# dkohlsdorf/audio_pattern_discovery

Measured on AMD Instinct MI355X. Metric: DTW cell-updates/sec (whole node), higher is better.
Workload: dtype f32

## Files before the change

audio_pattern_discovery_amd/csrc/dtw_systolic.h:

```cpp
#pragma once
#include <type_traits>

#ifndef APD_ABLATE
#define APD_ABLATE 0
#endif

#include "dtw_common.h"

namespace apd {

typedef float apd_f32x4 __attribute__((ext_vector_type(4)));
constexpr uint32_t kNoFrame = 0xFFFFFF00u;

template <int D>
__device__ __forceinline__ void load_frame(float (&dst)[D], __amdgpu_buffer_rsrc_t rsrc, uint32_t byte_off)
{
    constexpr int DP4 = (D + 3) / 4;
#pragma unroll
    for (int q = 0; q < DP4; ++q) {
        const apd_f32x4 t = __builtin_bit_cast(apd_f32x4, __builtin_amdgcn_raw_buffer_load_b128(rsrc, byte_off + 16u * q, 0, 0));
        if (4 * q + 0 < D) dst[4 * q + 0] = t.x;
        if (4 * q + 1 < D) dst[4 * q + 1] = t.y;
        if (4 * q + 2 < D) dst[4 * q + 2] = t.z;
        if (4 * q + 3 < D) dst[4 * q + 3] = t.w;
    }
}

template <int D>
__device__ __forceinline__ void load_frame_dwords(float (&dst)[D], __amdgpu_buffer_rsrc_t rsrc, uint32_t byte_off)
{
#pragma unroll
    for (int k = 0; k < D; ++k)
        dst[k] = __builtin_bit_cast(float, __builtin_amdgcn_raw_buffer_load_b32(rsrc, byte_off + 4u * k, 0, 0));
}

template <int D, int DN>
__device__ __forceinline__ float frame_dist(const float (&x)[DN], const float (&y)[DN])
{
    float t = x[0] - y[0];
    float acc = t * t;
#pragma unroll
    for (int k = 1; k < D; ++k) {
        t = x[k] - y[k];
        acc = __builtin_fmaf(t, t, acc);
    }
    if (APD_ABLATE & 1) return acc;
    return __builtin_amdgcn_sqrtf(acc);
}

template <int D, int DN>
__device__ __forceinline__ float frame_sq_strict(const float (&x)[DN], const float (&y)[DN])
{
    float t = x[0] - y[0];
    float acc = t * t;
#pragma unroll
    for (int k = 1; k < D; ++k) {
        t = x[k] - y[k];
        const float sq = t * t;
        acc = acc + sq;
    }
    return acc;
}
template <int D, int DN>
__device__ __forceinline__ float frame_dist_strict(const float (&x)[DN], const float (&y)[DN])
{
    return __builtin_sqrtf(frame_sq_strict<D, DN>(x, y));
}

template <int D>
__device__ __forceinline__ float frame_sq_expanded_pre(const float (&xm)[D + 1], const float (&y)[D + 1])
{
    float acc = xm[D] + y[D];
#pragma unroll
    for (int k = 0; k < D; ++k) acc = __builtin_fmaf(xm[k], y[k], acc);
    return acc;
}
template <int D>
__device__ __forceinline__ void prescale_row_piece(apd_f32x4 &v, int piece)
{
    const bool np = piece == D / 4;
    v.x = (np && D % 4 == 0) ? v.x : -2.0f * v.x;
    v.y = (np && D % 4 == 1) ? v.y : -2.0f * v.y;
    v.z = (np && D % 4 == 2) ? v.z : -2.0f * v.z;
    v.w = (np && D % 4 == 3) ? v.w : -2.0f * v.w;
}
template <int D>
__device__ __forceinline__ float frame_sq_exact_pre(const float (&xm)[D + 1], const float (&y)[D + 1])
{
    float t = __builtin_fmaf(-0.5f, xm[0], -y[0]);
    float acc = t * t;
#pragma unroll
    for (int k = 1; k < D; ++k) {
        t = __builtin_fmaf(-0.5f, xm[k], -y[k]);
        acc = __builtin_fmaf(t, t, acc);
    }
    return acc;
}
template <int C, int G, bool UNIFORM_PEN>
__device__ __forceinline__ void dp_rows_step(float (&prev1)[C], float (&prev2)[C], const float (&d)[C], const bool (&g1)[C],
                                             const bool (&g2)[C], float del, float ins, float mat, int gl)
{
    float left1 = group_from_lower_wrap<G>(prev1[C - 1], APD_INF, gl);
    float left2 = group_from_lower_wrap<G>(prev2[C - 1], APD_INF, gl);
    float upr1 = APD_INF, upr2 = APD_INF;
#pragma unroll
    for (int c = 0; c < C; ++c) {
        if (APD_ABLATE & 2) { prev1[c] += d[c]; prev2[c] -= d[c]; continue; }
        const float up1 = (c < C - 1) ? prev1[(c + 1) % C] : upr1;
        const float up2 = (c < C - 1) ? prev2[(c + 1) % C] : upr2;
        const float r1 = select_node<UNIFORM_PEN>(left1, up1, prev1[c], d[c], del, ins, mat, (APD_ABLATE & 16) ? false : g1[c]);
        const float r2 = select_node<UNIFORM_PEN>(up2, left2, prev2[c], d[c], del, ins, mat, (APD_ABLATE & 16) ? false : g2[c]);
        prev1[c] = r1; prev2[c] = r2;
        left1 = r1; left2 = r2;
        if (c == 0) {
            upr1 = group_from_upper_wrap<G>(r1, APD_INF, gl);
            upr2 = group_from_upper_wrap<G>(r2, APD_INF, gl);
        }
    }
}
template <int C>
__device__ __forceinline__ void slow_phase_captures(float (&prev1)[C], float (&prev2)[C], float &res1, float &res2, int tau, int gl,
                                                    int tau_cap, int cw, int cstar)
{
    if (tau == gl) {
#pragma unroll
        for (int c = 0; c < C; ++c) if (c == cw) { prev1[c] = 0.0f; prev2[c] = 0.0f; }
    }
    if (tau == tau_cap) {
#pragma unroll
        for (int c = 0; c < C; ++c) if (c == cstar) { res1 = prev1[c]; res2 = prev2[c]; }
    }
}
template <int D, int C, int G, bool UNIFORM_PEN, bool HYBRID>
__global__ __launch_bounds__(256) void dtw_fused_systolic(const AlignLaunch L)
{
    static_assert(C >= 2 && (64 % G) == 0, "bad geometry");
    if (L.d_nonfinite != nullptr && *L.d_nonfinite != 0u) return;
    constexpr int DN = D + 1;
    constexpr int DP = (DN + 3) & ~3;
    constexpr int PPW = 64 / G;
    constexpr int WPT = kSlotsPerTile / (4 * PPW);
    const int lane = threadIdx.x & 63;
    const int gl = lane % G;
    const uint32_t xcd = blockIdx.x & 7u, q = blockIdx.x >> 3;
    const uint32_t tile = (q / WPT) * 8u + xcd;
    const uint32_t slot = ((q % WPT) * 4u + (threadIdx.x >> 6)) * PPW + lane / G;
    const PairInfo P = decode_pair(L, tile, slot);
    const bool special = P.valid && (P.n == 1 || P.m == 1);
    const bool sweep = P.valid && !special;
    if (__ballot(sweep) == 0ull) {
        if (special && gl == 0) { const float s = (P.n == 1 && P.m == 1) ? 0.0f : APD_INF; store_pair(L, tile, P, s, s); }
        return;
    }
    const int n = sweep ? P.n : 1, m = sweep ? P.m : 1, w = sweep ? P.w : 2;
    const __amdgpu_buffer_rsrc_t rsrc = __builtin_amdgcn_make_buffer_rsrc((void *)L.d_frames, 0, L.frames_bytes, 0x00020000);
    const uint32_t a_off = (uint32_t)(P.A - L.d_frames) * 4u, b_off = (uint32_t)(P.B - L.d_frames) * 4u;
    constexpr uint32_t FB = DP * 4u;
    float ins = L.band.ins, del = L.band.del, mat = L.band.mat;
    float tau_thr = L.tau, nmax_b = P.nmax_b;
    asm volatile("" : "+v"(ins), "+v"(del), "+v"(mat), "+v"(tau_thr), "+v"(nmax_b));
    constexpr int R = (G == 64) ? 128 : 64;
    constexpr int LPF = DP / 4;
    constexpr int FPF = 64 / LPF;
    constexpr int RS = DP + 4;
    constexpr int U_ROWS = ((C + 1) % 2 == 0) ? (C + 1) : 2 * (C + 1);
    __shared__ float xring_all[4][(R + U_ROWS) * RS];
    float *const xring = xring_all[threadIdx.x >> 6];
    const int lead = __builtin_ctzll(__ballot(sweep));
    const uint32_t a_off_w = __builtin_amdgcn_readlane(a_off, lead);
    const int n_w = __builtin_amdgcn_readlane(n, lead);
    const int u0 = C * gl;
    const int two_w = 2 * w;

    bool g1[C], g2[C];
#pragma unroll
    for (int c = 0; c < C; ++c) {
        const int u = u0 + c;
        g1[c] = u >= two_w;
        g2[c] = (u == 0) | (u > two_w);
    }
    const int cw = w - u0;
    const int ustar = (m - 1) - (n - 1) + w;
    const int cstar = ustar - u0;
    const int tau_cap = (n - 1) + gl;

    const int g_act = (two_w + 1 + C - 1) / C;
    int my_total = sweep ? (n - 1) + g_act : 0;
    int my_min = sweep ? (n - 1) : 0x7fffffff;
    int total = 0, min_rows = 0x7fffffff;
#pragma unroll
    for (int g = 0; g < PPW; ++g) {
        total = max(total, __builtin_amdgcn_readlane(my_total, g * G));
        min_rows = min(min_rows, __builtin_amdgcn_readlane(my_min, g * G));
    }
    constexpr int S = C + 1;
    constexpr int U = (S % 2 == 0) ? S : 2 * S;
    static_assert(U == U_ROWS, "ring copy sized for another unroll");
    constexpr bool MASKED_FETCH = HYBRID && (G == 32 || G == 8) && !(APD_ABLATE & 512);
    const int total_r = ((total + U - 1) / U) * U;
    int a_steps = G;
    if (UNIFORM_PEN && !HYBRID) {
        int w_max = 0;
#pragma unroll
        for (int g = 0; g < PPW; ++g) w_max = max(w_max, __builtin_amdgcn_readlane(w, g * G));
        a_steps = max(G, w_max + 1);
    }
    const int a_end = min(((a_steps + U - 1) / U) * U, total_r);
    const int b_end = min(max((min_rows / U) * U, a_end), total_r);

    float prev1[C], prev2[C];
#pragma unroll
    for (int c = 0; c < C; ++c) { prev1[c] = APD_INF; prev2[c] = APD_INF; }
    float res1 = 0.0f, res2 = 0.0f;

    float yf[S][DN];
#pragma unroll
    for (int c = 0; c < C; ++c) {
        const int j = u0 - gl + c - w;
        const int idx = (j >= 1) ? (min(j, m) - 1) : (HYBRID ? m : m + 1);
        load_frame<DN>(yf[c], rsrc, b_off + (uint32_t)idx * FB);
    }
#pragma unroll
    for (int k = 0; k < DN; ++k) yf[C][k] = 0.0f;
    if (HYBRID && !MASKED_FETCH && !(APD_ABLATE & 8)) {
        const int jt = 1 + (C - 1) * G - w;
        const uint32_t yo = b_off + (uint32_t)((jt >= 1) ? (min(jt, m) - 1) : m) * FB;
        load_frame<DN>(yf[C], rsrc, gl == G - 1 ? yo : kNoFrame);
    }
    constexpr int NFILL = (U + FPF - 1) / FPF;
    const int fill_f = lane / LPF, fill_q = lane % LPF;
    auto fill_load = [&](int first_row, apd_f32x4 (&regs)[NFILL]) __attribute__((always_inline)) {
#pragma unroll
        for (int f = 0; f < NFILL; ++f) {
            const int fi = f * FPF + fill_f;
            const bool act = (fill_f < FPF) & (fi < U);
            const uint32_t off = a_off_w + (uint32_t)(min(first_row + fi, n_w) - 1) * FB + 16u * fill_q;
            regs[f] = __builtin_bit_cast(apd_f32x4, __builtin_amdgcn_raw_buffer_load_b128(rsrc, act ? off : kNoFrame, 0, 0));
        }
    };
    auto fill_store = [&](int first_row, const apd_f32x4 (&regs)[NFILL]) __attribute__((always_inline)) {
#pragma unroll
        for (int f = 0; f < NFILL; ++f) {
            const int fi = f * FPF + fill_f;
            if ((fill_f < FPF) & (fi < U)) {
                apd_f32x4 v = regs[f];
                if (HYBRID) prescale_row_piece<D>(v, fill_q);
                const int slot = (first_row + fi) & (R - 1);
                *reinterpret_cast<apd_f32x4 *>(&xring[slot * RS + 4 * fill_q]) = v;
                if (slot < U) *reinterpret_cast<apd_f32x4 *>(&xring[(slot + R) * RS + 4 * fill_q]) = v;
            }
        }
    };
    for (int e = lane; e < G * DP; e += 64) {
        const int slot = (-(e / DP)) & (R - 1);
        const float v = HYBRID ? ((e % DP) == D ? APD_INF : 0.0f) : -APD_INF;
        xring[slot * RS + (e % DP)] = v;
        if (slot < U) xring[(slot + R) * RS + (e % DP)] = v;
    }
    {
        apd_f32x4 regs[NFILL];
        fill_load(1, regs);
        fill_store(1, regs);
    }
    asm volatile("" ::: "memory");
    auto read_row = [&](float (&dst)[DN], int row) __attribute__((always_inline)) {
        const float *p = &xring[(row & (R - 1)) * RS];
#pragma unroll
        for (int q = 0; q < LPF; ++q) {
            const apd_f32x4 t = *reinterpret_cast<const apd_f32x4 *>(p + 4 * q);
            if (4 * q + 0 < DN) dst[4 * q + 0] = t.x;
            if (4 * q + 1 < DN) dst[4 * q + 1] = t.y;
            if (4 * q + 2 < DN) dst[4 * q + 2] = t.z;
            if (4 * q + 3 < DN) dst[4 * q + 3] = t.w;
        }
    };
    auto read_row_at = [&](float (&dst)[DN], const float *p) __attribute__((always_inline)) {
#pragma unroll
        for (int q = 0; q < LPF; ++q) {
            const apd_f32x4 t = *reinterpret_cast<const apd_f32x4 *>(p + 4 * q);
            if (4 * q + 0 < DN) dst[4 * q + 0] = t.x;
            if (4 * q + 1 < DN) dst[4 * q + 1] = t.y;
            if (4 * q + 2 < DN) dst[4 * q + 2] = t.z;
            if (4 * q + 3 < DN) dst[4 * q + 3] = t.w;
        }
    };
    constexpr int NX = HYBRID ? 1 : 2;
    float xs[NX][DN];
    read_row(xs[0], 0 - gl);
#pragma unroll
    for (int k = 0; k < DN; ++k) xs[NX - 1][k] = (NX == 1) ? xs[0][k] : 0.0f;
    constexpr bool PIPE = (APD_ABLATE & 32) != 0;
    float dn[C];
#pragma unroll
    for (int c = 0; c < C; ++c) dn[c] = (PIPE && !HYBRID && c < C - 1) ? frame_dist_strict<D, DN>(xs[0], yf[c]) : 0.0f;

    auto advance_window = [&](int q) __attribute__((always_inline)) {
        const int r = q % S, e = (r + C) % S;
#pragma unroll
        for (int k = 0; k < (HYBRID ? DN : D); ++k) {
            if (APD_ABLATE & 4) { yf[e][k] = yf[(r + 1) % S][k] + yf[e][k]; continue; }
            yf[e][k] = MASKED_FETCH ? dpp_move<(G == 8) ? 0x101 : 0x130>(yf[(r + 1) % S][k], yf[e][k])
                                    : group_from_upper<G>(yf[(r + 1) % S][k], yf[e][k], gl);
        }
    };
    auto macro_steps = [&](int tau_begin, int tau_end, auto slow_tag) __attribute__((always_inline)) {
        constexpr bool SLOW = decltype(slow_tag)::value;
        uint32_t yo_cur = kNoFrame, yo_cap = kNoFrame, yo_step = 0u;
        if (!SLOW && gl == G - 1) {
            yo_cap = b_off + (uint32_t)(m - 1) * FB;
            yo_cur = min(b_off + (uint32_t)(tau_begin + ((HYBRID && !MASKED_FETCH) ? 1 : 0) + (C - 1) * G - w) * FB, yo_cap);
            yo_step = FB;
        }
        auto fetch_column = [&](float (&dst)[DN], int t) __attribute__((always_inline)) {
            if (APD_ABLATE & 8) return;
            if (SLOW) {
                const int jt = t + 1 + (C - 1) * G - w;
                const uint32_t yo = b_off + (uint32_t)((jt >= 1) ? (min(jt, m) - 1) : (HYBRID ? m : m + 1)) * FB;
                load_frame<DN>(dst, rsrc, gl == G - 1 ? yo : kNoFrame);
            } else {
                load_frame<DN>(dst, rsrc, yo_cur);
                yo_cur = min(yo_cur + yo_step, yo_cap);
            }
        };
        for (int tau0 = tau_begin; tau0 < tau_end; tau0 += U) {
            apd_f32x4 fill_regs[NFILL];
            fill_load(tau0 + U + 1, fill_regs);
            const float *const xrows = &xring[((tau0 + 1 - gl) & (R - 1)) * RS];
#pragma unroll
            for (int q = 0; q < U; ++q) {
                const int tau = tau0 + q;
                const int r = q % S;
                const int xa = HYBRID ? 0 : (q & 1), xb = HYBRID ? 0 : (xa ^ 1);
                const int e = (r + C) % S;
                if (!HYBRID) {
                    fetch_column(yf[e], tau);
                    read_row_at(xs[xb], xrows + q * RS);
                }
                float d[C];
                if (HYBRID) {
#pragma unroll
                    for (int c = 0; c < C; ++c) {
                        d[c] = frame_sq_expanded_pre<D>(xs[xa], yf[(r + c) % S]);
                    }
                    float dmin = d[0];
#pragma unroll
                    for (int c = 1; c + 1 < C; c += 2) dmin = __builtin_fminf(__builtin_fminf(dmin, d[c]), d[c + 1]);
                    if (C % 2 == 0) dmin = __builtin_fminf(dmin, d[C - 1]);
                    const bool any = (APD_ABLATE & 128) ? false : dmin < (xs[xa][D] + nmax_b) * tau_thr;
                    advance_window(q);
                    if (MASKED_FETCH) {
                        if (gl == G - 1) fetch_column(yf[e], tau);
                    }
                    if (__builtin_expect(__ballot(any) != 0ull, 0)) {
                        float nx = xs[xa][D];
                        asm volatile("" : "+v"(nx));
#pragma unroll
                        for (int c = 0; c < C; ++c) {
                            const float sc = nx + yf[(r + c) % S][D];
                            const float ex = frame_sq_exact_pre<D>(xs[xa], yf[(r + c) % S]);
                            d[c] = (d[c] < sc * tau_thr) ? ex : d[c];
                        }
                    }
                    if (!MASKED_FETCH) fetch_column(yf[r], tau + 1);
#pragma unroll
                    for (int c = 0; c < C; ++c) d[c] = (APD_ABLATE & 1) ? d[c] : __builtin_amdgcn_sqrtf(d[c]);
                    read_row_at(xs[0], xrows + q * RS);
                } else if (UNIFORM_PEN && !SLOW && !PIPE) {
                    float d2[C];
#pragma unroll
                    for (int c = 0; c < C; ++c) d2[c] = frame_sq_strict<D, DN>(xs[xa], yf[(r + c) % S]);
                    float dmin = d2[0];
#pragma unroll
                    for (int c = 1; c + 1 < C; c += 2) dmin = __builtin_fminf(__builtin_fminf(dmin, d2[c]), d2[c + 1]);
                    if (C % 2 == 0) dmin = __builtin_fminf(dmin, d2[C - 1]);
                    if (__builtin_expect(__ballot(!(dmin >= 0x1p-96f)) != 0ull, 0)) {
#pragma unroll
                        for (int c = 0; c < C; ++c) d[c] = __builtin_sqrtf(d2[c]);
                    } else {
#pragma unroll
                        for (int c = 0; c < C; ++c) d[c] = sqrt_rn_finite(d2[c]);
                    }
                } else {
#pragma unroll
                    for (int c = 0; c < C; ++c)
                        d[c] = (UNIFORM_PEN && PIPE && c < C - 1) ? dn[c] : frame_dist_strict<D, DN>(xs[xa], yf[(r + c) % S]);
                    if (PIPE) {
#pragma unroll
                        for (int c = 0; c < C - 1; ++c) dn[c] = frame_dist_strict<D, DN>(xs[xb], yf[(r + 1 + c) % S]);
                    }
                }
                dp_rows_step<C, G, UNIFORM_PEN>(prev1, prev2, d, g1, g2, del, ins, mat, gl);
                if (SLOW) slow_phase_captures<C>(prev1, prev2, res1, res2, tau, gl, tau_cap, cw, cstar);
                if (!HYBRID) advance_window(q);
            }
            fill_store(tau0 + U + 1, fill_regs);
            asm volatile("" ::: "memory");
        }
    };
    macro_steps(0, a_end, std::true_type{});
    macro_steps(a_end, b_end, std::false_type{});
    macro_steps(b_end, total_r, std::true_type{});

    if (P.valid && gl == (sweep ? ustar / C : 0)) {
        if (sweep) {
            const float denom = (float)(n + m);
            store_pair(L, tile, P, res1 / denom, res2 / denom);
        } else {
            const float s = (P.n == 1 && P.m == 1) ? 0.0f : APD_INF;
            store_pair(L, tile, P, s, s);
        }
    }
}

typedef float apd_f32x2 __attribute__((ext_vector_type(2)));
template <int DN>
__device__ __forceinline__ void read_frame_lds(float (&dst)[DN], const float *p)
{
    constexpr int FULL = DN / 4, TAIL = DN % 4;
#pragma unroll
    for (int k = 0; k < FULL; ++k) {
        const apd_f32x4 t = *reinterpret_cast<const apd_f32x4 *>(p + 4 * k);
        dst[4 * k + 0] = t.x; dst[4 * k + 1] = t.y; dst[4 * k + 2] = t.z; dst[4 * k + 3] = t.w;
    }
    if (TAIL >= 2) {
        const apd_f32x2 t = *reinterpret_cast<const apd_f32x2 *>(p + 4 * FULL);
        dst[4 * FULL + 0] = t.x; dst[4 * FULL + 1] = t.y;
    }
    if (TAIL == 1) dst[4 * FULL] = p[4 * FULL];
    if (TAIL == 3) dst[4 * FULL + 2] = p[4 * FULL + 2];
}

constexpr int shared_column_ring_floats(int rc, int u, int dp) { return (((rc + u) * dp + ((rc + u + 7) / 8) * 4) * 4 + 255) / 256 * 64; }

template <int D, int C, int G>
__global__ __launch_bounds__(256) void dtw_fused_systolic_shared(const AlignLaunch L)
{
    static_assert(C >= 2 && G == 16, "one ring per wavefront: four lane groups");
    if (L.d_nonfinite != nullptr && *L.d_nonfinite != 0u) return;
    constexpr int DN = D + 1;
    constexpr int DP = (DN + 3) & ~3;
    constexpr int PPW = 64 / G;
    constexpr int WPT = kSlotsPerTile / (4 * PPW);
    constexpr int S = C + 1;
    constexpr int U = shared_column_unroll(C);
    constexpr int RC = shared_column_ring_frames(G, C);
    constexpr int R = 64;
    constexpr int LPF = DP / 4;
    constexpr int FPF = 64 / LPF;
    constexpr int RS = DP + 4;
    constexpr uint32_t FB = DP * 4u;
    constexpr int XRING = (R + U) * RS;
    constexpr int CRING = shared_column_ring_floats(RC, U, DP);
    static_assert(FPF >= U && RC % 8 == 0, "one wave-wide load per fill");
    static_assert(RC >= (G - 1) * (C - 1) + 2 * U + (int)shared_column_slack(KernelGeom{KernelGeom::SharedColumns, G, C}),
                  "ring too short for the spread of w the tile plan admits");
    extern __shared__ __attribute__((aligned(16))) float apd_shared_lds[];
    const int lane = threadIdx.x & 63, wave = threadIdx.x >> 6;
    const int gl = lane % G;
    float *const xring = apd_shared_lds + wave * XRING;
    float *const crings = apd_shared_lds + 4 * XRING;
    int *const wg_words = reinterpret_cast<int *>(crings + PPW * CRING);
    const uint32_t xcd = blockIdx.x & 7u, q = blockIdx.x >> 3;
    const uint32_t tile = (q / WPT) * 8u + xcd;
    const uint32_t sub = q % WPT;
    const uint32_t slot = ((sub / 4u) * 4u + wave) * kTile + (sub % 4u) * 4u + lane / G;
    const PairInfo P = decode_pair(L, tile, slot);
    const bool special = P.valid && (P.n == 1 || P.m == 1);
    const bool sweep = P.valid && !special;
    const int n = sweep ? P.n : 1, m = sweep ? P.m : 1, w = sweep ? P.w : 2;
    const int u0 = C * gl;
    const int two_w = 2 * w;
    const int g_act = (two_w + 1 + C - 1) / C;
    int my_total = sweep ? (n - 1) + g_act : 0;
    int my_min = sweep ? (n - 1) : 0x7fffffff;
    int my_w = sweep ? w : 0x7fffffff;
    int total = 0, min_rows = 0x7fffffff, w_lo = 0x7fffffff;
#pragma unroll
    for (int g = 0; g < PPW; ++g) {
        total = max(total, __builtin_amdgcn_readlane(my_total, g * G));
        min_rows = min(min_rows, __builtin_amdgcn_readlane(my_min, g * G));
        w_lo = min(w_lo, __builtin_amdgcn_readlane(my_w, g * G));
    }
    if (lane == 0) { wg_words[2 * wave] = total; wg_words[2 * wave + 1] = w_lo; }
    __syncthreads();
    total = 0; w_lo = 0x7fffffff;
#pragma unroll
    for (int k = 0; k < 4; ++k) { total = max(total, wg_words[2 * k]); w_lo = min(w_lo, wg_words[2 * k + 1]); }
    if (total == 0) {
        if (special && gl == 0) { const float s = (P.n == 1 && P.m == 1) ? 0.0f : APD_INF; store_pair(L, tile, P, s, s); }
        return;
    }
    const __amdgpu_buffer_rsrc_t rsrc = __builtin_amdgcn_make_buffer_rsrc((void *)L.d_frames, 0, L.frames_bytes, 0x00020000);
    const uint32_t a_off = (uint32_t)(P.A - L.d_frames) * 4u, b_off = (uint32_t)(P.B - L.d_frames) * 4u;
    float ins = L.band.ins, del = L.band.del, mat = L.band.mat;
    float tau_thr = L.tau, nmax_b = P.nmax_b;
    asm volatile("" : "+v"(ins), "+v"(del), "+v"(mat), "+v"(tau_thr), "+v"(nmax_b));
    const unsigned long long sweeping = __ballot(sweep);
    const int lead = sweeping ? __builtin_ctzll(sweeping) : 0;
    const uint32_t a_off_w = sweeping ? __builtin_amdgcn_readlane(a_off, lead) : 0u;
    const int n_w = sweeping ? __builtin_amdgcn_readlane(n, lead) : 1;
    uint32_t cb_off = 0u;
    int cm = 0;
    bool cvalid = false;
    {
        const uint4 t = L.d_tiles[tile];
        const uint32_t b = t.y * kTile + (sub % 4u) * 4u + wave;
        if (b < L.n_seq) {
            const uint32_t ob = L.d_seq_off[b];
            cm = (int)(L.d_seq_off[b + 1] - ob) - 2;
            cb_off = ob * L.dpad * 4u;
            cvalid = true;
        }
    }

    bool g1[C], g2[C];
#pragma unroll
    for (int c = 0; c < C; ++c) {
        const int u = u0 + c;
        g1[c] = u >= two_w;
        g2[c] = (u == 0) | (u > two_w);
    }
    const int cw = w - u0;
    const int ustar = (m - 1) - (n - 1) + w;
    const int cstar = ustar - u0;
    const int tau_cap = (n - 1) + gl;
    const int total_r = ((total + U - 1) / U) * U;
    const int a_end = min(((G + U - 1) / U) * U, total_r);
    const int b_end = min(max((min_rows / U) * U, a_end), total_r);

    float prev1[C], prev2[C];
#pragma unroll
    for (int c = 0; c < C; ++c) { prev1[c] = APD_INF; prev2[c] = APD_INF; }
    float res1 = 0.0f, res2 = 0.0f;

    float yf[S][DN];
#pragma unroll
    for (int c = 0; c < C; ++c) {
        const int j = u0 - gl + c - w;
        const int idx = (j >= 1) ? (min(j, m) - 1) : m;
        load_frame<DN>(yf[c], rsrc, b_off + (uint32_t)idx * FB);
    }
#pragma unroll
    for (int k = 0; k < DN; ++k) yf[C][k] = 0.0f;

    constexpr int NFILL = (U + FPF - 1) / FPF;
    const int fill_f = lane / LPF, fill_q = lane % LPF;
    const bool fill_act = (fill_f < FPF) & (fill_f < U);
    auto fill_load = [&](int first_row, apd_f32x4 (&regs)[NFILL]) __attribute__((always_inline)) {
        const uint32_t off = a_off_w + (uint32_t)(min(first_row + fill_f, n_w) - 1) * FB + 16u * fill_q;
        regs[0] = __builtin_bit_cast(apd_f32x4, __builtin_amdgcn_raw_buffer_load_b128(rsrc, fill_act ? off : kNoFrame, 0, 0));
    };
    auto fill_store = [&](int first_row, const apd_f32x4 (&regs)[NFILL]) __attribute__((always_inline)) {
        if (fill_act) {
            apd_f32x4 v = regs[0];
            prescale_row_piece<D>(v, fill_q);
            const int rslot = (first_row + fill_f) & (R - 1);
            *reinterpret_cast<apd_f32x4 *>(&xring[rslot * RS + 4 * fill_q]) = v;
            if (rslot < U) *reinterpret_cast<apd_f32x4 *>(&xring[(rslot + R) * RS + 4 * fill_q]) = v;
        }
    };
    for (int e = lane; e < G * DP; e += 64) {
        const int rslot = (-(e / DP)) & (R - 1);
        const float v = (e % DP) == D ? APD_INF : 0.0f;
        xring[rslot * RS + (e % DP)] = v;
        if (rslot < U) xring[(rslot + R) * RS + (e % DP)] = v;
    }
    {
        apd_f32x4 regs[NFILL];
        fill_load(1, regs);
        fill_store(1, regs);
    }
    float *const cring_fill = crings + wave * CRING;
    const int col_hi0 = U + (C - 1) * G - w_lo;
    auto ring_slot = [](int j) { return (j + 64 * RC) % RC; };
    auto ring_at = [](auto *ring, uint32_t p) { return ring + p * DP + ((p >> 3) << 2); };
    auto col_load = [&](int j, bool act) __attribute__((always_inline)) {
        const int idx = (j >= 1) ? (min(j, cm) - 1) : cm;
        const uint32_t off = cb_off + (uint32_t)idx * FB + 16u * fill_q;
        return __builtin_bit_cast(apd_f32x4, __builtin_amdgcn_raw_buffer_load_b128(rsrc, (act & cvalid) ? off : kNoFrame, 0, 0));
    };
    for (int j0 = col_hi0 - RC + 1; j0 <= col_hi0; j0 += FPF) {
        const int j = j0 + fill_f;
        const bool act = (fill_f < FPF) & (j <= col_hi0);
        const apd_f32x4 v = col_load(j, act);
        const uint32_t ps = (uint32_t)ring_slot(j);
        if (act) *reinterpret_cast<apd_f32x4 *>(ring_at(cring_fill, ps) + 4 * fill_q) = v;
        if (act && ps < (uint32_t)U) *reinterpret_cast<apd_f32x4 *>(ring_at(cring_fill, ps + RC) + 4 * fill_q) = v;
    }
    uint32_t pf = (uint32_t)ring_slot(col_hi0 + 1 + fill_f);
    const float *const cring_read = crings + (lane / G) * CRING;
    uint32_t pr = (uint32_t)ring_slot(1 + (C - 1) * (gl + 1) - w);
    auto read_col = [&](float (&dst)[DN], const float *block_base, int q) __attribute__((always_inline)) {
        read_frame_lds<DN>(dst, block_base + q * DP + (((pr + (uint32_t)q) >> 3) << 2));
    };
    __syncthreads();
    auto read_row_at = [&](float (&dst)[DN], const float *p) __attribute__((always_inline)) { read_frame_lds<DN>(dst, p); };
    float xs[DN];
    read_row_at(xs, &xring[((0 - gl) & (R - 1)) * RS]);

    auto macro_steps = [&](int tau_begin, int tau_end, auto slow_tag) __attribute__((always_inline)) {
        constexpr bool SLOW = decltype(slow_tag)::value;
        for (int tau0 = tau_begin; tau0 < tau_end; tau0 += U) {
            apd_f32x4 fill_regs[NFILL];
            fill_load(tau0 + U + 1, fill_regs);
            const apd_f32x4 col_regs = col_load(tau0 + col_hi0 + 1 + fill_f, fill_act);
            const float *const xrows = &xring[((tau0 + 1 - gl) & (R - 1)) * RS];
            const float *const ycols = cring_read + pr * DP;
#pragma unroll
            for (int q = 0; q < U; ++q) {
                const int tau = tau0 + q;
                const int r = q % S;
                const int e = (r + C) % S;
                float d[C];
#pragma unroll
                for (int c = 0; c < C; ++c) d[c] = frame_sq_expanded_pre<D>(xs, yf[(r + c) % S]);
                float dmin = d[0];
#pragma unroll
                for (int c = 1; c + 1 < C; c += 2) dmin = __builtin_fminf(__builtin_fminf(dmin, d[c]), d[c + 1]);
                if (C % 2 == 0) dmin = __builtin_fminf(dmin, d[C - 1]);
                const bool any = dmin < (xs[D] + nmax_b) * tau_thr;
                read_col(yf[e], ycols, q);
                if (__builtin_expect(__ballot(any) != 0ull, 0)) {
                    float nx = xs[D];
                    asm volatile("" : "+v"(nx));
#pragma unroll
                    for (int c = 0; c < C; ++c) {
                        const float sc = nx + yf[(r + c) % S][D];
                        const float ex = frame_sq_exact_pre<D>(xs, yf[(r + c) % S]);
                        d[c] = (d[c] < sc * tau_thr) ? ex : d[c];
                    }
                }
#pragma unroll
                for (int c = 0; c < C; ++c) d[c] = __builtin_amdgcn_sqrtf(d[c]);
                read_row_at(xs, xrows + q * RS);
                dp_rows_step<C, G, true>(prev1, prev2, d, g1, g2, del, ins, mat, gl);
                if (SLOW) slow_phase_captures<C>(prev1, prev2, res1, res2, tau, gl, tau_cap, cw, cstar);
            }
            fill_store(tau0 + U + 1, fill_regs);
            if (fill_act) *reinterpret_cast<apd_f32x4 *>(ring_at(cring_fill, pf) + 4 * fill_q) = col_regs;
            if (fill_act && pf < (uint32_t)U) *reinterpret_cast<apd_f32x4 *>(ring_at(cring_fill, pf + RC) + 4 * fill_q) = col_regs;
            pf = min(pf + (uint32_t)U, pf + (uint32_t)U - (uint32_t)RC);
            pr = min(pr + (uint32_t)U, pr + (uint32_t)U - (uint32_t)RC);
            __syncthreads();
        }
    };
    macro_steps(0, a_end, std::true_type{});
    macro_steps(a_end, b_end, std::false_type{});
    macro_steps(b_end, total_r, std::true_type{});

    if (P.valid && gl == (sweep ? ustar / C : 0)) {
        if (sweep) {
            const float denom = (float)(n + m);
            store_pair(L, tile, P, res1 / denom, res2 / denom);
        } else {
            const float s = (P.n == 1 && P.m == 1) ? 0.0f : APD_INF;
            store_pair(L, tile, P, s, s);
        }
    }
}

template <int D, int C, int G>
constexpr size_t shared_columns_lds_bytes()
{
    constexpr int DP = (D + 1 + 3) & ~3, U = shared_column_unroll(C), RC = shared_column_ring_frames(G, C);
    constexpr int XRING = (64 + U) * (DP + 4), CRING = shared_column_ring_floats(RC, U, DP);
    return (size_t)(4 * XRING + (64 / G) * CRING + 8) * sizeof(float);
}
template <int D, int C, int G>
static hipError_t launch_shared_columns_kernel(const AlignLaunch &L, hipStream_t stream)
{
    constexpr int WPT = kSlotsPerTile / (4 * (64 / G));
    constexpr size_t lds = shared_columns_lds_bytes<D, C, G>();
    static_assert(lds <= 80 * 1024, "two workgroups per CU");
    static bool granted[64] = {};
    int dev = 0;
    if (hipError_t e = hipGetDevice(&dev); e != hipSuccess) return e;
    if (dev < 0 || dev >= 64 || !granted[dev]) {
        const hipError_t e = hipFuncSetAttribute(reinterpret_cast<const void *>(dtw_fused_systolic_shared<D, C, G>),
                                                 hipFuncAttributeMaxDynamicSharedMemorySize, (int)lds);
        if (e != hipSuccess) return e;
        if (dev >= 0 && dev < 64) granted[dev] = true;
    }
    const uint32_t tiles8 = (L.n_tiles + 7u) / 8u * 8u;
    hipLaunchKernelGGL((dtw_fused_systolic_shared<D, C, G>), dim3(tiles8 * WPT), dim3(256), lds, stream, L);
    return hipSuccess;
}

template <int D, int C, int G, bool UNIFORM_PEN, bool HYBRID>
static void launch_systolic_kernel(const AlignLaunch &L, hipStream_t stream)
{
    constexpr int PPW = 64 / G;
    constexpr int WPT = kSlotsPerTile / (4 * PPW);
    const uint32_t tiles8 = (L.n_tiles + 7u) / 8u * 8u;
    hipLaunchKernelGGL((dtw_fused_systolic<D, C, G, UNIFORM_PEN, HYBRID>), dim3(tiles8 * WPT), dim3(256), 0, stream, L);
}

#ifdef APD_SYSTOLIC_STRICT_UNIT
template <int D>
bool launch_systolic_strict(const AlignLaunch &L, KernelGeom g, hipStream_t stream)
{
#define APD_CASE(GG, CC) if constexpr (geom_instantiated(KernelGeom{KernelGeom::Systolic, GG, CC}, D)) { \
        if (g == KernelGeom{KernelGeom::Systolic, GG, CC}) { launch_systolic_kernel<D, CC, GG, true, false>(L, stream); return true; } }
    APD_SYSTOLIC_GEOMS(APD_CASE)
#undef APD_CASE
    return false;
}
#else
template <int D>
bool launch_systolic(const AlignLaunch &L, KernelGeom g, hipStream_t stream)
{
    const bool unit = L.band.ins == 1.0f && L.band.del == 1.0f && L.band.mat == 1.0f;
    if (g.family == KernelGeom::SharedColumns) {
        if (!(unit && L.hybrid)) return false;
#define APD_CASE(GG, CC) if constexpr (geom_instantiated(KernelGeom{KernelGeom::SharedColumns, GG, CC}, D)) { \
        if (g == KernelGeom{KernelGeom::SharedColumns, GG, CC}) return launch_shared_columns_kernel<D, CC, GG>(L, stream) == hipSuccess; }
        APD_SHARED_COLUMN_GEOMS(APD_CASE)
#undef APD_CASE
        return false;
    }
    if (unit && !L.hybrid) return launch_systolic_strict<D>(L, g, stream);
#define APD_CASE(GG, CC) if constexpr (geom_instantiated(KernelGeom{KernelGeom::Systolic, GG, CC}, D)) { \
        if (g == KernelGeom{KernelGeom::Systolic, GG, CC}) { \
            if (!unit) launch_systolic_kernel<D, CC, GG, false, false>(L, stream); else launch_systolic_kernel<D, CC, GG, true, true>(L, stream); \
            return true; } }
    APD_SYSTOLIC_GEOMS(APD_CASE)
#undef APD_CASE
    return false;
}
#endif

}
```

Baseline: 3131 billion.

## Software-pipeline distance computation one step ahead and interleave with DP recurrence

Restructures the systolic DTW inner loop so the squared distances for the next step are computed inside the current step's DP update, interleaved per column with the select_node recurrence. The ballot threshold test also moves one step ahead. The ring-padding offset in LDS column reads becomes a precomputed base plus compare-selects. The end-of-block stores and barrier move inside the last unrolled iteration. The fast phase adds explicit sched_group_barrier ordering to interleave LDS reads with VALU work. All of this aims to hide LDS latency and the dependency chain, at the cost of more live registers and a re-read of the previous row on the rare exact-distance path.

```diff
diff --git a/audio_pattern_discovery_amd/csrc/dtw_systolic.h b/audio_pattern_discovery_amd/csrc/dtw_systolic.h
--- a/audio_pattern_discovery_amd/csrc/dtw_systolic.h
+++ b/audio_pattern_discovery_amd/csrc/dtw_systolic.h
@@ -590,13 +590,46 @@
     uint32_t pf = (uint32_t)ring_slot(col_hi0 + 1 + fill_f);
     const float *const cring_read = crings + (lane / G) * CRING;
     uint32_t pr = (uint32_t)ring_slot(1 + (C - 1) * (gl + 1) - w);
-    auto read_col = [&](float (&dst)[DN], const float *block_base, int q) __attribute__((always_inline)) {
-        read_frame_lds<DN>(dst, block_base + q * DP + (((pr + (uint32_t)q) >> 3) << 2));
+    static_assert(U <= 16, "at most two steps of the padding term per block");
+    auto read_col = [&](float (&dst)[DN], const float *base, uint32_t q_hi, int q) __attribute__((always_inline)) {
+        const float *p = base;
+        if (q >= 1) p = (uint32_t)q >= q_hi ? base + 4 : p;
+        if (q >= 9) p = (uint32_t)q >= q_hi + 8u ? base + 8 : p;
+        read_frame_lds<DN>(dst, p + q * DP);
     };
     __syncthreads();
     auto read_row_at = [&](float (&dst)[DN], const float *p) __attribute__((always_inline)) { read_frame_lds<DN>(dst, p); };
-    float xs[DN];
-    read_row_at(xs, &xring[((0 - gl) & (R - 1)) * RS]);
+    auto row_at = [&](int row) { return &xring[(row & (R - 1)) * RS]; };
+    auto min_of = [](const float (&v)[C]) __attribute__((always_inline)) {
+        float lo = v[0];
+#pragma unroll
+        for (int c = 1; c + 1 < C; c += 2) lo = __builtin_fminf(__builtin_fminf(lo, v[c]), v[c + 1]);
+        if (C % 2 == 0) lo = __builtin_fminf(lo, v[C - 1]);
+        return lo;
+    };
+    float xs[DN], d2[C];
+    unsigned long long hit;
+    const float *xrows = row_at(1 - gl);
+    {
+        read_row_at(xs, row_at(0 - gl));
+#pragma unroll
+        for (int c = 0; c < C; ++c) d2[c] = frame_sq_expanded_pre<D>(xs, yf[c]);
+        const float thr = (xs[D] + nmax_b) * tau_thr;
+        read_row_at(xs, xrows);
+        hit = __ballot(min_of(d2) < thr);
+    }
+    auto pipeline_order = [&]() __attribute__((always_inline)) {
+        constexpr int N1 = (D + 1) / 3, N2 = (D + 1 - N1) / 2, N3 = D + 1 - N1 - N2;
+#pragma unroll
+        for (int c = 0; c < C; ++c) {
+            __builtin_amdgcn_sched_group_barrier(0x400, 1, 0);
+            if (c == 0) __builtin_amdgcn_sched_group_barrier(0x2, 2 + 2, 0); else __builtin_amdgcn_sched_group_barrier(0x2, 2 + N1, 0);
+            __builtin_amdgcn_sched_group_barrier(0x4, 1, 0);
+            if (c == 0) __builtin_amdgcn_sched_group_barrier(0x2, 4, 0); else __builtin_amdgcn_sched_group_barrier(0x2, 4 + N2, 0);
+            __builtin_amdgcn_sched_group_barrier(0x4, 1, 0);
+            if (c == 0) __builtin_amdgcn_sched_group_barrier(0x2, 2 + 2, 0); else __builtin_amdgcn_sched_group_barrier(0x2, 2 + N3, 0);
+        }
+    };
 
     auto macro_steps = [&](int tau_begin, int tau_end, auto slow_tag) __attribute__((always_inline)) {
         constexpr bool SLOW = decltype(slow_tag)::value;
@@ -604,44 +637,61 @@
             apd_f32x4 fill_regs[NFILL];
             fill_load(tau0 + U + 1, fill_regs);
             const apd_f32x4 col_regs = col_load(tau0 + col_hi0 + 1 + fill_f, fill_act);
-            const float *const xrows = &xring[((tau0 + 1 - gl) & (R - 1)) * RS];
-            const float *const ycols = cring_read + pr * DP;
+            const float *const ycols = cring_read + pr * DP + ((pr >> 3) << 2);
+            const uint32_t q_hi = 8u - (pr & 7u);
 #pragma unroll
             for (int q = 0; q < U; ++q) {
                 const int tau = tau0 + q;
                 const int r = q % S;
                 const int e = (r + C) % S;
-                float d[C];
-#pragma unroll
-                for (int c = 0; c < C; ++c) d[c] = frame_sq_expanded_pre<D>(xs, yf[(r + c) % S]);
-                float dmin = d[0];
-#pragma unroll
-                for (int c = 1; c + 1 < C; c += 2) dmin = __builtin_fminf(__builtin_fminf(dmin, d[c]), d[c + 1]);
-                if (C % 2 == 0) dmin = __builtin_fminf(dmin, d[C - 1]);
-                const bool any = dmin < (xs[D] + nmax_b) * tau_thr;
-                read_col(yf[e], ycols, q);
-                if (__builtin_expect(__ballot(any) != 0ull, 0)) {
+                read_col(yf[e], ycols, q_hi, q);
+                if (__builtin_expect(hit != 0ull, 0)) {
+                    read_row_at(xs, row_at(tau - gl));
                     float nx = xs[D];
                     asm volatile("" : "+v"(nx));
 #pragma unroll
                     for (int c = 0; c < C; ++c) {
                         const float sc = nx + yf[(r + c) % S][D];
                         const float ex = frame_sq_exact_pre<D>(xs, yf[(r + c) % S]);
-                        d[c] = (d[c] < sc * tau_thr) ? ex : d[c];
+                        d2[c] = (d2[c] < sc * tau_thr) ? ex : d2[c];
+                    }
+                    read_row_at(xs, xrows + q * RS);
+                }
+                float left1 = group_from_lower_wrap<G>(prev1[C - 1], APD_INF, gl);
+                float left2 = group_from_lower_wrap<G>(prev2[C - 1], APD_INF, gl);
+                float upr1 = APD_INF, upr2 = APD_INF;
+#pragma unroll
+                for (int c = 0; c < C; ++c) {
+                    const float dc = __builtin_amdgcn_sqrtf(d2[c]);
+                    if (c > 0) d2[c - 1] = frame_sq_expanded_pre<D>(xs, yf[(r + c) % S]);
+                    const float up1 = (c < C - 1) ? prev1[c + 1] : upr1;
+                    const float up2 = (c < C - 1) ? prev2[c + 1] : upr2;
+                    const float r1 = select_node<true>(left1, up1, prev1[c], dc, del, ins, mat, g1[c]);
+                    const float r2 = select_node<true>(up2, left2, prev2[c], dc, del, ins, mat, g2[c]);
+                    prev1[c] = r1; prev2[c] = r2;
+                    left1 = r1; left2 = r2;
+                    if (c == 0) {
+                        upr1 = group_from_upper_wrap<G>(r1, APD_INF, gl);
+                        upr2 = group_from_upper_wrap<G>(r2, APD_INF, gl);
                     }
                 }
-#pragma unroll
-                for (int c = 0; c < C; ++c) d[c] = __builtin_amdgcn_sqrtf(d[c]);
-                read_row_at(xs, xrows + q * RS);
-                dp_rows_step<C, G, true>(prev1, prev2, d, g1, g2, del, ins, mat, gl);
+                d2[C - 1] = frame_sq_expanded_pre<D>(xs, yf[e]);
+                const float thr = (xs[D] + nmax_b) * tau_thr;
+                const float dmin = min_of(d2);
+                if (!SLOW) pipeline_order();
+                if (q == U - 1) {
+                    fill_store(tau0 + U + 1, fill_regs);
+                    if (fill_act) *reinterpret_cast<apd_f32x4 *>(ring_at(cring_fill, pf) + 4 * fill_q) = col_regs;
+                    if (fill_act && pf < (uint32_t)U) *reinterpret_cast<apd_f32x4 *>(ring_at(cring_fill, pf + RC) + 4 * fill_q) = col_regs;
+                    pf = min(pf + (uint32_t)U, pf + (uint32_t)U - (uint32_t)RC);
+                    pr = min(pr + (uint32_t)U, pr + (uint32_t)U - (uint32_t)RC);
+                    __syncthreads();
+                    xrows = row_at(tau0 + U + 1 - gl);
+                }
+                read_row_at(xs, q == U - 1 ? xrows : xrows + (q + 1) * RS);
+                hit = __ballot(dmin < thr);
                 if (SLOW) slow_phase_captures<C>(prev1, prev2, res1, res2, tau, gl, tau_cap, cw, cstar);
             }
-            fill_store(tau0 + U + 1, fill_regs);
-            if (fill_act) *reinterpret_cast<apd_f32x4 *>(ring_at(cring_fill, pf) + 4 * fill_q) = col_regs;
-            if (fill_act && pf < (uint32_t)U) *reinterpret_cast<apd_f32x4 *>(ring_at(cring_fill, pf + RC) + 4 * fill_q) = col_regs;
-            pf = min(pf + (uint32_t)U, pf + (uint32_t)U - (uint32_t)RC);
-            pr = min(pr + (uint32_t)U, pr + (uint32_t)U - (uint32_t)RC);
-            __syncthreads();
         }
     };
     macro_steps(0, a_end, std::true_type{});
```

Result: slower. 3009 billion (-3.9%).
